# facebookresearch/audio2photoreal

Hardware: NVIDIA B200
Metric: motion-frames/sec full p_sample_loop (body, 1000 steps, T=600) (higher is better)
Workload: dtype bf16x2 split (fp32-equivalent), fp32 accumulate

## Files before the change

audio2photoreal_b200/csrc/engine.cu:

```cuda
#include <cuda_runtime.h>
#include <stdlib.h>
#include <map>
#include <string>
#include <vector>

#include "../../include/a2p_b200.h"
#include "attention_simt.cuh"
#include "common.cuh"
#include "elementwise.cuh"
#include "sgemm.cuh"
#include "umma_gemm.cuh"
#include "umma_attention.cuh"
#include "umma_chain.cuh"
#include "umma_attention2.cuh"
#include "umma_attention_short.cuh"

using namespace a2p;

namespace {

constexpr int MAXL = 16;
constexpr int TCN_PAD = 24;
const int TCN_DIL[6] = {1, 2, 3, 1, 2, 3};

struct AttnW { const float *in_w, *in_b, *out_w, *out_b; };
struct LayerW {
  AttnW sa, ca, c2;
  const float *l1w, *l1b, *l2w, *l2b;
  const float *n1w, *n1b, *n2w, *n2b, *n2aw, *n2ab, *n3w, *n3b;
};

struct CondSet {
  bool set = false;
  int Bc = 0, S = 0, S2 = 0;
  float* base = nullptr;
  const float* hidden = nullptr;
};

struct GraphKey {
  int B, T, kind, n_steps, clip, mask;
  const void *coeffs, *ts, *scale, *x, *pred, *noise, *ws;
  const void *kv0, *kv1;
  unsigned long long seed; long long row0; int rng;
  int units;
  int pipes;
  bool operator==(const GraphKey& o) const {
    return B == o.B && T == o.T && kind == o.kind && n_steps == o.n_steps && clip == o.clip && mask == o.mask &&
           coeffs == o.coeffs && ts == o.ts && scale == o.scale && x == o.x && pred == o.pred && noise == o.noise &&
           ws == o.ws && kv0 == o.kv0 && kv1 == o.kv1 && seed == o.seed && row0 == o.row0 && rng == o.rng && units == o.units && pipes == o.pipes;
  }
};

}

struct a2p_denoiser {
  a2p_model_cfg cfg{};
  int dh = 0, nf = 0;
  bool bound = false;
  LayerW lw[MAXL]{};
  const float *time_w1, *time_b1, *time_w2, *time_b2, *time_w3, *time_b3;
  const float *normc_w, *normc_b, *inp_w, *inp_b, *fin_w, *fin_b, *fconv_w, *fconv_b;
  struct EncLayerW { const float *n1w, *n1b, *n2w, *n2b, *in_w, *in_b, *out_w, *out_b, *l1w, *l1b, *l2w, *l2b; };
  struct EncW {
    const float *cp_w = nullptr, *cp_b = nullptr;
    const float *p0w = nullptr, *p0b = nullptr, *p1w = nullptr, *p1b = nullptr, *p3w = nullptr, *p3b = nullptr;
    const float *fp_w = nullptr, *fp_b = nullptr, *fn_w = nullptr, *fn_b = nullptr;
    EncLayerW enc[2]{};
    int feat_dim = 0;
    bool ok = false;
  } encw;
  const float* conv_b[6];
  const float* time_freqs;
  float *film_w = nullptr, *film_b = nullptr, *ttk_w = nullptr, *ttk_b = nullptr, *ttv_w = nullptr, *ttv_b = nullptr;
  float* conv_w[6]{};
  float* conv_t[6]{};
  float2* rope_tab = nullptr;
  std::map<const float*, __nv_bfloat16*> wplanes;
  std::map<const float*, long long> wnumel;
  int num_sms = 148;
  int attn_skew_ns = 0;
  CondSet cond[2];
  int64_t launches = 0;
  int64_t graph_nodes = 0;
  static constexpr int MAXG = 4;
  cudaGraphExec_t gexec[MAXG] = {};
  int n_gexec = 0;
  cudaStream_t group_stream[MAXG] = {};
  cudaEvent_t ev_gstart = nullptr, ev_gdone[MAXG] = {}, ev_gfork[MAXG] = {};
  cudaStream_t cap_stream = nullptr;
  static constexpr int MAXU = 8;
  cudaStream_t cond_stream[MAXU] = {};
  cudaEvent_t ev_fork[MAXU] = {}, ev_join[MAXU] = {};
  cudaStream_t unit_stream[MAXU] = {};
  cudaEvent_t ev_ujoin[MAXU] = {};
  cudaEvent_t ev_bfork = nullptr;
  GraphKey gkey{};
  bool gvalid = false;
};

namespace {

struct PackedLayout {
  size_t film_w, film_b, ttk_w, ttk_b, ttv_w, ttv_b, conv_w[6], conv_t[6], rope, planes, planes_bytes, total;
};
size_t split_weight_elems(const a2p_model_cfg& c) {
  const size_t D = c.D, FF = c.FF, C = c.C;
  size_t per_layer = 2 * (3 * D * D + D * D) + 2 * FF * D + (c.fmt == A2P_FMT_POSE ? 4 * D * D : 0);
  size_t conv = 0;
  if (c.fmt == A2P_FMT_POSE) {
    const size_t cm = C > 256 ? C : 256;
    conv = 3 * (cm * C * 2 + C * C * 4) + C * C;
  }
  return per_layer * c.L + 2 * D * C + conv;
}
PackedLayout packed_layout(const a2p_model_cfg& c) {
  PackedLayout p{};
  size_t off = 0;
  auto take = [&](size_t nfloats) { size_t o = off; off = align_up(off + nfloats * 4, 256); return o; };
  const int nf = c.fmt == A2P_FMT_POSE ? 4 : 3;
  p.film_w = take((size_t)c.L * nf * 2 * c.D * c.D);
  p.film_b = take((size_t)c.L * nf * 2 * c.D);
  p.ttk_w = take((size_t)c.L * c.D * c.D);
  p.ttk_b = take((size_t)c.L * c.D);
  p.ttv_w = take((size_t)c.L * c.D * c.D);
  p.ttv_b = take((size_t)c.L * c.D);
  if (c.fmt == A2P_FMT_POSE) {
    const int cm = c.C > 256 ? c.C : 256;
    const int chans[6][2] = {{cm, c.C}, {c.C, cm}, {c.C, c.C}, {c.C, c.C}, {c.C, c.C}, {c.C, c.C}};
    for (int i = 0; i < 6; ++i) p.conv_w[i] = take((size_t)chans[i][0] * chans[i][1] * 3);
    for (int i = 0; i < 6; ++i) p.conv_t[i] = take((size_t)chans[i][0] * chans[i][1] * 3);
  }
  p.rope = take((size_t)c.max_pos * (c.D / 2) * 2);
  p.planes = off;
  p.planes_bytes = c.split_terms > 0 ? align_up(split_weight_elems(c) * 2 * c.split_terms + 64 * 256, 256) : 0;
  off += p.planes_bytes;
  p.total = off;
  return p;
}

struct KvLayout {
  size_t per_layer, ka, va, k2, v2, hidden, total;
  size_t kaP, vtaP, k2P, vt2P;
  size_t Sp, S2p;
};
KvLayout kv_layout(const a2p_model_cfg& c, int Bc, int S, int S2) {
  KvLayout k{};
  size_t a = (size_t)Bc * S * c.D, b = (size_t)Bc * S2 * c.D;
  k.ka = 0; k.va = a; k.k2 = 2 * a; k.v2 = 2 * a + b;
  k.per_layer = 2 * a + 2 * b;
  k.Sp = align_up((size_t)S, 8); k.S2p = align_up((size_t)(S2 > 0 ? S2 : 1), 8);
  if (c.split_terms > 0) {
    const size_t P = c.split_terms;
    auto take = [&](size_t bf16s) { size_t o = k.per_layer; k.per_layer += align_up(bf16s / 2 + 1, 64); return o; };
    k.per_layer = align_up(k.per_layer, 64);
    k.kaP = take(P * Bc * S * c.D);
    k.vtaP = take(P * c.D * Bc * k.Sp);
    k.k2P = take(P * (b ? b : 1));
    k.vt2P = take(P * c.D * Bc * k.S2p);
  }
  k.hidden = k.per_layer * c.L;
  k.total = k.hidden + (size_t)Bc * c.D;
  return k;
}

struct WsLayout {
  size_t counter, e, th, mt, ttok, tt, ttr, ktt, vtt, film, xin, x, h, hr, qkv, att, u, out, tcnA, tcnB, tcnC, total;
  size_t hP, hrP, attP, uP, xinP;
  size_t tcnUP, tcnVP;
// ... 160 lines not shown
const float* find(const std::map<std::string, std::pair<const float*, int64_t>>& m, const std::string& k, int64_t numel,
                  std::string& err) {
  auto it = m.find(k);
  if (it == m.end()) { if (err.empty()) err = "missing weight '" + k + "'"; return nullptr; }
  if (numel >= 0 && it->second.second != numel) {
    if (err.empty()) err = "weight '" + k + "' has " + std::to_string(it->second.second) + " elements, expected " + std::to_string(numel);
    return nullptr;
  }
  return it->second.first;
}

int attn2_variant() {
  static int v = -1;
  if (v < 0) v = getenv("A2P_ATTN2") ? atoi(getenv("A2P_ATTN2")) : 2;
  return v;
}

int branch_groups(int B) {
  const char* e = getenv("A2P_BRANCH_GROUPS");
  const int v = e ? atoi(e) : ((B >= 4 && B <= 16) ? 2 : 1);
  return v >= 4 ? 4 : (v >= 2 ? 2 : 1);
}
bool branch_streams_disabled() { return getenv("A2P_NO_BRANCH_STREAMS") != nullptr; }
int branch_stagger() {
  static int v = -1;
  if (v < 0) { const char* e = getenv("A2P_BRANCH_STAGGER"); v = e ? atoi(e) : 0; if (v < 0) v = 0; }
  return v;
}

int chain_priority() {
  static int v = 1 << 30;
  if (v == (1 << 30)) { const char* e = getenv("A2P_CHAIN_PRIO"); v = e ? atoi(e) : 0; }
  return v;
}

bool chain_disabled() {
  static int v = -1;
  if (v < 0) v = getenv("A2P_NO_CHAIN") ? 1 : 0;
  return v == 1;
}

int check_cfg(const a2p_model_cfg* c) {
  if (!c) A2P_FAIL("null cfg");
  if (c->fmt != A2P_FMT_POSE && c->fmt != A2P_FMT_FACE) A2P_FAIL("cfg.fmt must be 0 (pose) or 1 (face)");
  if (c->D != 256 && c->D != 512) A2P_FAIL("cfg.D=%d unsupported (256 or 512)", c->D);
  if (c->H <= 0 || c->D % c->H) A2P_FAIL("cfg.H=%d does not divide D=%d", c->H, c->D);
  int dh = c->D / c->H;
  if (dh != 32 && dh != 64) A2P_FAIL("head dim %d unsupported (32 or 64)", dh);
  if (c->L <= 0 || c->L > MAXL) A2P_FAIL("cfg.L=%d out of range", c->L);
  if (c->C % 8 || c->FF % 8) A2P_FAIL("cfg.C/FF must be multiples of 8");
  if (c->fmt == A2P_FMT_POSE && c->S2 <= 0) A2P_FAIL("pose needs S2 > 0");
  if (c->fmt == A2P_FMT_FACE && c->S2 != 0) A2P_FAIL("face must have S2 == 0");
  if (c->split_terms < 0 || c->split_terms > 3) A2P_FAIL("split_terms=%d must be 0 (exact fp32) or 1..3 bf16 planes", c->split_terms);
  if (c->max_pos < 2) A2P_FAIL("cfg.max_pos too small");
  return 0;
}

int forward_core(Ctx& c, int B, int T, const float* xin, const long long* ts, const int* counter, int mask, char* wsb,
                 const float** x0_cond, const float** x0_uncond, long long* x0_sample_stride, int b0 = 0, int B_total = 0) {
  if (B_total <= 0) B_total = B;
  a2p_denoiser* h = c.h;
  const a2p_model_cfg& cf = h->cfg;
  const int D = cf.D, L = cf.L, C = cf.C, nf = h->nf, H = cf.H, dh = h->dh;
  const int nb = (mask == A2P_MASK_BOTH) ? 2 : 1;
  const int R = nb * B;
  const int br0 = (mask == A2P_MASK_UNCOND) ? 1 : 0;
// ... 379 lines not shown
      a.V = a.K;
      a.V.base[0] = c0.base + k0.per_layer * l + k0.v2;
      a.V.base[1] = c1.base ? c1.base + k1.per_layer * l + k1.v2 : nullptr;
      a.kv_ld = D; a.S_main = S2; a.S_extra = 0;
      a.O = att; a.o_ld = D; a.o_sample_stride = sT; a.T = T; a.H = H; a.R = R; a.scale_log2e = scale_log2e;
      c.cat = CAT_ATT_CROSS2;
      c.begin(); A2P_TRY(launch_attn_simt(a, dh, st)); c.end();
      c.cat = CAT_PROJ;
      h->launches++;
      A2P_TRY(film_gemm(c, att, D, R * T, lw.c2.out_w, lw.c2.out_b, D, D, x, D, film, film_ld, fo + 2 * 2 * D, D, T));
    }
    c.cat = CAT_FFN;
    { int _c = c.cat; c.cat = CAT_LN; c.begin(); A2P_TRY(launch_ln_rope(D, x, D, lw.n3w, lw.n3b, hh, nullptr, D, h->rope_tab, T, 0, R * T, st)); c.end(); c.cat = _c; }
    h->launches++;
    A2P_TRY(gemm(c, hh, D, R * T, lw.l1w, D, lw.l1b, cf.FF, D, u, cf.FF, EPI_GELU));
    A2P_TRY(film_gemm(c, u, cf.FF, R * T, lw.l2w, lw.l2b, D, cf.FF, x, D, film, film_ld, fo + (nf - 1) * 2 * D, D, T));
  }
  c.cat = CAT_IO_TCN;
  if (P > 0 && cf.fmt == A2P_FMT_POSE) {
    const int cm = C > 256 ? C : 256;
    const int Pl = T + TCN_PAD, Mp = R * Pl;
    __nv_bfloat16* U = reinterpret_cast<__nv_bfloat16*>(wsb + w.tcnUP);
    __nv_bfloat16* V = reinterpret_cast<__nv_bfloat16*>(wsb + w.tcnVP);
    float *X = F(w.tcnA), *Y = F(w.tcnC);
    c.cat = CAT_IO_TCN;
    if (!chain) {
      A2P_TRY(launch_split_planes(P, x, D, hP, pstrideD, MT, D, 1.f, st));
      A2P_CUDA(cudaMemset2DAsync(U, (size_t)Pl * C * 2, 0, (size_t)TCN_PAD * C * 2, (size_t)P * R, st));
      h->launches += 2;
      TcGemmParams g{};
      g.Cp = U; g.cp_plane_stride = (long long)Mp * C; g.ldcp = C; g.remap_rps = T; g.remap_pad = TCN_PAD;
      A2P_TRY(tc_gemm(c, hP, MT, D, h->fin_w, 0, C, h->fin_b, TC_PLANES, g));
    }
    struct St { __nv_bfloat16* in; int cin; __nv_bfloat16* outp; int cout; float* f32; const float* skip; };
    St stg[6] = {{U, C, V, cm, nullptr, nullptr}, {V, cm, U, C, X, nullptr}, {U, C, V, C, Y, X},
                 {V, C, U, C, X, Y},              {U, C, V, C, Y, X},        {V, C, U, C, nullptr, Y}};
    for (int i = 0; i < 6; ++i) {
      TcGemmParams g{};
      g.taps = 3; g.dil = TCN_DIL[i]; g.slope = 0.2f;
      g.Cp = stg[i].outp; g.cp_plane_stride = (long long)Mp * stg[i].cout; g.ldcp = stg[i].cout;
      g.C = stg[i].f32; g.ldc = stg[i].cout;
      g.skip = stg[i].skip; g.ldskip = stg[i].cout;
      A2P_TRY(tc_gemm(c, stg[i].in, Mp, stg[i].cin, h->conv_t[i], 0, stg[i].cout, h->conv_b[i], TC_LRELU_PLANES, g));
    }
    {
      TcGemmParams g{};
      g.C = Y; g.ldc = C;
      A2P_TRY(tc_gemm(c, U, Mp, C, h->fconv_w, 0, C, h->fconv_b, TC_F32, g));
    }
    *x0_sample_stride = (long long)Pl * C;
    const float* o0 = Y + (size_t)TCN_PAD * C;
    *x0_cond = (mask & A2P_MASK_COND) ? o0 : nullptr;
    *x0_uncond = (mask == A2P_MASK_BOTH) ? o0 + (size_t)B * Pl * C : (mask == A2P_MASK_UNCOND ? o0 : nullptr);
    return 0;
  }
  if (P > 0) {
    A2P_TRY(launch_split_planes(P, x, D, hP, pstrideD, MT, D, 1.f, st));
    h->launches++;
    TcGemmParams g{};
    g.C = out; g.ldc = C;
    A2P_TRY(tc_gemm(c, hP, MT, D, h->fin_w, 0, C, h->fin_b, TC_F32, g));
  } else {
    A2P_TRY(gemm(c, x, D, R * T, h->fin_w, D, h->fin_b, C, D, out, C));
  }
  if (cf.fmt == A2P_FMT_POSE) {
    const int cm = C > 256 ? C : 256;
    const int P = T + TCN_PAD;
    float *A = F(w.tcnA), *Bf = F(w.tcnB), *Cc = F(w.tcnC);
    long long total = (long long)R * P * (C / 4);
    pad_copy_kernel<<<(unsigned)((total + 255) / 256), 256, 0, st>>>(out, A, T, TCN_PAD, C / 4, total);
    h->launches++;
    struct Stage { const float* in; int cin; float* outp; int cout; bool skip; };
    Stage stg[6] = {{A, C, Bf, cm, false}, {Bf, cm, A, C, false}, {A, C, Cc, C, true},
                    {Cc, C, A, C, true},   {A, C, Cc, C, true},   {Cc, C, A, C, true}};
    for (int i = 0; i < 6; ++i) {
      GemmParams ex{};
      ex.taps = 3; ex.dil = TCN_DIL[i]; ex.Kc = stg[i].cin; ex.slope = 0.2f;
      ex.skip = stg[i].in; ex.ldskip = stg[i].cin;
      const bool skip = stg[i].skip && stg[i].cin == stg[i].cout;
      A2P_TRY(gemm(c, stg[i].in, stg[i].cin, R * P, h->conv_w[i], 3LL * stg[i].cin, h->conv_b[i], stg[i].cout, 3 * stg[i].cin,
                   stg[i].outp, stg[i].cout, skip ? EPI_LRELU_SKIPAVG : EPI_LRELU, &ex));
// ... 183 lines not shown
      int tot = (int)(chans[i][0] * chans[i][1] * 3);
      permute_conv_w_kernel<<<ceil_div(tot, 256), 256, 0, st>>>(cw, h->conv_w[i], (int)chans[i][0], (int)chans[i][1]);
      permute_conv_w_tapmajor_kernel<<<ceil_div(tot, 256), 256, 0, st>>>(cw, h->conv_t[i], (int)chans[i][0], (int)chans[i][1]);
    }
    h->fconv_w = W("final_conv.weight", C * C); h->fconv_b = W("final_conv.bias", C);
  }
  if (!err.empty()) A2P_FAIL("bind_weights: %s", err.c_str());
  h->wplanes.clear(); h->wnumel.clear();
  if (cf.split_terms > 0) {
    __nv_bfloat16* cur = reinterpret_cast<__nv_bfloat16*>(pb + pl.planes);
    const __nv_bfloat16* endp = reinterpret_cast<__nv_bfloat16*>(pb + pl.planes + pl.planes_bytes);
    auto split_w = [&](const float* wsrc, long long rows, long long cols) -> int {
      const long long numel = rows * cols;
      if (cur + numel * cf.split_terms > endp) A2P_FAIL("bind_weights: plane arena overflow");
      A2P_TRY(launch_split_planes(cf.split_terms, wsrc, cols, cur, numel, rows, (int)cols, 1.f, st));
      h->wplanes[wsrc] = cur; h->wnumel[wsrc] = numel;
      cur += align_up((size_t)numel * cf.split_terms, 64);
      return 0;
    };
    for (int l = 0; l < cf.L; ++l) {
      const LayerW& lw = h->lw[l];
      A2P_TRY(split_w(lw.sa.in_w, 3 * D, D)); A2P_TRY(split_w(lw.sa.out_w, D, D));
      A2P_TRY(split_w(lw.ca.in_w, 3 * D, D)); A2P_TRY(split_w(lw.ca.out_w, D, D));
      if (cf.fmt == A2P_FMT_POSE) { A2P_TRY(split_w(lw.c2.in_w, 3 * D, D)); A2P_TRY(split_w(lw.c2.out_w, D, D)); }
      A2P_TRY(split_w(lw.l1w, FF, D)); A2P_TRY(split_w(lw.l2w, D, FF));
    }
    A2P_TRY(split_w(h->inp_w, D, C)); A2P_TRY(split_w(h->fin_w, C, D));
    if (cf.fmt == A2P_FMT_POSE) {
      const int64_t cm = C > 256 ? C : 256;
      const int64_t chans[6][2] = {{cm, C}, {C, cm}, {C, C}, {C, C}, {C, C}, {C, C}};
      for (int i = 0; i < 6; ++i) A2P_TRY(split_w(h->conv_t[i], 3 * chans[i][0], chans[i][1]));
      A2P_TRY(split_w(h->fconv_w, C, C));
    }
    A2P_TRY(init_umma_gemm());
    A2P_TRY(init_umma_attn());
    A2P_TRY(init_umma_chain());
    A2P_TRY(init_umma_attn2());
    A2P_TRY(init_umma_attn_short());
  }
  {
    int dev = 0;
    cudaGetDevice(&dev);
    cudaDeviceGetAttribute(&h->num_sms, cudaDevAttrMultiProcessorCount, dev);
  }
  rope_table_kernel<<<ceil_div(cf.max_pos * (int)(D / 2), 256), 256, 0, st>>>(freqs, h->rope_tab, cf.max_pos, (int)(D / 2));
  A2P_CUDA(cudaGetLastError());
  h->bound = true;
  h->gvalid = false;
  return 0;
}

size_t a2p_kv_cache_bytes(const a2p_model_cfg* cfg, int Bc, int S) {
  if (check_cfg(cfg) || Bc <= 0 || S <= 0) return 0;
  return kv_layout(*cfg, Bc, S, cfg->S2).total * sizeof(float);
}

size_t a2p_conditioning_workspace_bytes(const a2p_model_cfg* cfg, int Bc, int S) {
  if (check_cfg(cfg) || Bc <= 0 || S <= 0) return 0;
  const size_t D = cfg->D;
  return (2 * align_up((size_t)Bc * S * D, 64) + align_up((size_t)Bc * (cfg->S2 > 0 ? cfg->S2 : 1) * D, 64)) * sizeof(float) + 512;
}

size_t a2p_workspace_bytes(const a2p_model_cfg* cfg, int B, int T) {
  if (check_cfg(cfg) || B <= 0 || T <= 0) return 0;
  const size_t one = ws_layout(*cfg, B, T).total;
  if (!(cfg->split_terms == 2 && cfg->D == 256)) return one;
// ... 486 lines not shown
```

audio2photoreal_b200/csrc/testing.cu:

```cuda
#include <cuda_runtime.h>
#include <stdlib.h>
#include <string>
#include <vector>

#include "../../include/a2p_b200.h"
#include "attention_simt.cuh"
#include "common.cuh"
#include "elementwise.cuh"
#include "sgemm.cuh"
#include "umma_gemm.cuh"
#include "umma_attention.cuh"
#include "umma_chain.cuh"
#include "umma_attention2.cuh"
#include "umma_attention_short.cuh"
#include "umma_microbench.cuh"
#include "../../include/a2p_b200_testing.h"

using namespace a2p;

extern "C" {

const char* a2p_test_last_error(void) { return a2p::last_error().c_str(); }

size_t a2p_test_tc_gemm_scratch_bytes(int M, int N, int K, int taps) {
  return ((size_t)3 * M * K + (size_t)3 * taps * N * K) * 2 + 1024;
}

int a2p_test_tc_gemm(int terms, int M, int N, int K, int taps, int dil, const float* A, const float* W, const float* bias,
                     float* C, void* scratch, size_t scratch_bytes, int iters, float* ms_out, void* stream) {
  if (scratch_bytes < a2p_test_tc_gemm_scratch_bytes(M, N, K, taps)) A2P_FAIL("test_tc_gemm: scratch too small");
  cudaStream_t st = (cudaStream_t)stream;
  A2P_TRY(init_umma_gemm());
  int dev = 0, sms = 148;
  cudaGetDevice(&dev);
  cudaDeviceGetAttribute(&sms, cudaDevAttrMultiProcessorCount, dev);
  __nv_bfloat16* Ap = (__nv_bfloat16*)scratch;
  __nv_bfloat16* Wp = Ap + align_up((size_t)3 * M * K, 64);
  A2P_TRY(launch_split_planes(terms, A, K, Ap, (long long)M * K, M, K, 1.f, st));
  A2P_TRY(launch_split_planes(terms, W, K, Wp, (long long)taps * N * K, (long long)taps * N, K, 1.f, st));
  TcOperands o{Ap, K, (long long)M * K, Wp, K, (long long)N * K};
  TcGemmParams p{};
  p.M = M; p.N = N; p.K = K; p.taps = taps; p.dil = dil; p.bias = bias; p.C = C; p.ldc = N; p.out_scale = 1.f;
  A2P_TRY(launch_umma_gemm(terms, o, p, TC_F32, sms, st));
  cudaEvent_t e0, e1;
  cudaEventCreate(&e0); cudaEventCreate(&e1);
  cudaEventRecord(e0, st);
  for (int i = 0; i < iters; ++i) A2P_TRY(launch_umma_gemm(terms, o, p, TC_F32, sms, st));
  cudaEventRecord(e1, st);
// ... 197 lines not shown
  cudaEvent_t e0, e1;
  cudaEventCreate(&e0); cudaEventCreate(&e1);
  cudaEventRecord(e0, st);
  for (int i = 0; i < iters; ++i) A2P_TRY(launch_attn_simt(a, dh, st));
  cudaEventRecord(e1, st);
  A2P_CUDA(cudaStreamSynchronize(st));
  float ms = 0.f;
  cudaEventElapsedTime(&ms, e0, e1);
  if (ms_out) *ms_out = iters > 0 ? ms / iters : 0.f;
  cudaEventDestroy(e0); cudaEventDestroy(e1);
  return 0;
}

int a2p_test_sgemm(int M, int N, int K, int taps, int dil, const float* A, const float* W, const float* bias, float* C,
                   int iters, float* ms_out, void* stream) {
  cudaStream_t st = (cudaStream_t)stream;
  GemmParams p{};
  p.A = A; p.lda = K; p.W = W; p.ldw = (long long)taps * K; p.bias = bias; p.C = C; p.ldc = N; p.M = M; p.N = N; p.K = taps * K;
  p.taps = taps; p.dil = dil; p.Kc = K; p.epi = EPI_BIAS;
  A2P_TRY(launch_sgemm(p, st));
  cudaEvent_t e0, e1;
  cudaEventCreate(&e0); cudaEventCreate(&e1);
  cudaEventRecord(e0, st);
  for (int i = 0; i < iters; ++i) A2P_TRY(launch_sgemm(p, st));
  cudaEventRecord(e1, st);
  A2P_CUDA(cudaStreamSynchronize(st));
  float ms = 0.f;
  cudaEventElapsedTime(&ms, e0, e1);
  if (ms_out) *ms_out = iters > 0 ? ms / iters : 0.f;
  cudaEventDestroy(e0); cudaEventDestroy(e1);
  return 0;
}

}
```

audio2photoreal_b200/csrc/umma.cuh:

```cuda
#pragma once
#include <cuda.h>
#include <cuda_bf16.h>
#include <cuda_runtime.h>
#include <stdint.h>

#include "common.cuh"

namespace a2p {
namespace umma {

__device__ __forceinline__ uint32_t smem_u32(const void* p) { return (uint32_t)__cvta_generic_to_shared(p); }

__device__ __forceinline__ void mbar_init(uint64_t* bar, uint32_t count) {
  asm volatile("mbarrier.init.shared::cta.b64 [%0], %1;" ::"r"(smem_u32(bar)), "r"(count));
}
__device__ __forceinline__ void fence_barrier_init() { asm volatile("fence.mbarrier_init.release.cluster;" ::: "memory"); }
__device__ __forceinline__ void fence_proxy_async() { asm volatile("fence.proxy.async.shared::cta;" ::: "memory"); }
__device__ __forceinline__ void mbar_expect_tx(uint64_t* bar, uint32_t bytes) {
  asm volatile("mbarrier.arrive.expect_tx.shared::cta.b64 _, [%0], %1;" ::"r"(smem_u32(bar)), "r"(bytes) : "memory");
}
__device__ __forceinline__ void mbar_arrive(uint64_t* bar) {
  asm volatile("mbarrier.arrive.shared::cta.b64 _, [%0];" ::"r"(smem_u32(bar)) : "memory");
}
__device__ __forceinline__ bool mbar_try_wait(uint64_t* bar, uint32_t parity) {
// ... 55 lines not shown
}
__device__ __forceinline__ void tma_load_3d_hint(const CUtensorMap* m, uint64_t* bar, void* dst, int c0, int c1, int c2, uint64_t pol) {
  asm volatile(
      "cp.async.bulk.tensor.3d.shared::cluster.global.mbarrier::complete_tx::bytes.L2::cache_hint [%0], [%1, {%3, %4, %5}], [%2], %6;"
      ::"r"(smem_u32(dst)), "l"(reinterpret_cast<uint64_t>(m)), "r"(smem_u32(bar)), "r"(c0), "r"(c1), "r"(c2), "l"(pol)
      : "memory");
}

template <int NCOLS>
__device__ __forceinline__ void tmem_alloc(uint32_t* slot_in_smem) {
  asm volatile("tcgen05.alloc.cta_group::1.sync.aligned.shared::cta.b32 [%0], %1;" ::"r"(smem_u32(slot_in_smem)), "n"(NCOLS));
  asm volatile("tcgen05.relinquish_alloc_permit.cta_group::1.sync.aligned;");
}
template <int NCOLS>
__device__ __forceinline__ void tmem_dealloc(uint32_t taddr) {
  asm volatile("tcgen05.dealloc.cta_group::1.sync.aligned.b32 %0, %1;" ::"r"(taddr), "n"(NCOLS));
}
__device__ __forceinline__ void fence_before() { asm volatile("tcgen05.fence::before_thread_sync;" ::: "memory"); }
__device__ __forceinline__ void fence_after() { asm volatile("tcgen05.fence::after_thread_sync;" ::: "memory"); }

__device__ __forceinline__ void tmem_ld32(uint32_t taddr, float* v) {
  uint32_t* r = reinterpret_cast<uint32_t*>(v);
  asm volatile(
      "tcgen05.ld.sync.aligned.32x32b.x32.b32 "
      "{%0, %1, %2, %3, %4, %5, %6, %7, %8, %9, %10, %11, %12, %13, %14, %15, "
      "%16, %17, %18, %19, %20, %21, %22, %23, %24, %25, %26, %27, %28, %29, %30, %31}, [%32];"
      : "=r"(r[0]), "=r"(r[1]), "=r"(r[2]), "=r"(r[3]), "=r"(r[4]), "=r"(r[5]), "=r"(r[6]), "=r"(r[7]), "=r"(r[8]),
        "=r"(r[9]), "=r"(r[10]), "=r"(r[11]), "=r"(r[12]), "=r"(r[13]), "=r"(r[14]), "=r"(r[15]), "=r"(r[16]),
        "=r"(r[17]), "=r"(r[18]), "=r"(r[19]), "=r"(r[20]), "=r"(r[21]), "=r"(r[22]), "=r"(r[23]), "=r"(r[24]),
        "=r"(r[25]), "=r"(r[26]), "=r"(r[27]), "=r"(r[28]), "=r"(r[29]), "=r"(r[30]), "=r"(r[31])
      : "r"(taddr));
}
__device__ __forceinline__ void tmem_ld_wait() { asm volatile("tcgen05.wait::ld.sync.aligned;" ::: "memory"); }

__device__ __forceinline__ uint64_t smem_desc_sw128(uint32_t saddr) {
  uint64_t d = 0;
  d |= (uint64_t)((saddr >> 4) & 0x3FFF);
  d |= (uint64_t)1 << 16;
  d |= (uint64_t)(1024 >> 4) << 32;
  d |= (uint64_t)1 << 46;
  d |= (uint64_t)2 << 61;
  return d;
}
constexpr uint32_t kDescHiSw128 = (uint32_t)(1024 >> 4) | (1u << 14) | (2u << 29);
__device__ __forceinline__ uint32_t desc_lo(uint32_t saddr) { return ((saddr >> 4) & 0x3FFFu) | (1u << 16); }
__device__ __forceinline__ uint64_t desc_make(uint32_t lo) { return ((uint64_t)kDescHiSw128 << 32) | (uint64_t)lo; }

__device__ __forceinline__ uint64_t smem_desc_sw64(uint32_t saddr) {
  uint64_t d = 0;
  d |= (uint64_t)((saddr >> 4) & 0x3FFF);
  d |= (uint64_t)1 << 16;
  d |= (uint64_t)(512 >> 4) << 32;
  d |= (uint64_t)1 << 46;
  d |= (uint64_t)4 << 61;
  return d;
}
__host__ __device__ constexpr uint32_t idesc_bf16_f32(int M, int N) {
  return (1u << 4) | (1u << 7) | (1u << 10) | ((uint32_t)(N >> 3) << 17) | ((uint32_t)(M >> 4) << 24);
}
__device__ __forceinline__ void mma_bf16(uint32_t tmem_d, uint64_t adesc, uint64_t bdesc, uint32_t idesc, uint32_t accumulate) {
  asm volatile(
      "{\n\t.reg .pred p;\n\t"
      "setp.ne.b32 p, %4, 0;\n\t"
      "tcgen05.mma.cta_group::1.kind::f16 [%0], %1, %2, %3, p;\n\t}"
      ::"r"(tmem_d), "l"(adesc), "l"(bdesc), "r"(idesc), "r"(accumulate)
      : "memory");
}
__device__ __forceinline__ void mma_commit(uint64_t* bar) {
  asm volatile("tcgen05.commit.cta_group::1.mbarrier::arrive::one.shared::cluster.b64 [%0];" ::"r"(smem_u32(bar)) : "memory");
}

__device__ __forceinline__ bool elect_one() {
  uint32_t pred;
  asm volatile(
      "{\n\t.reg .pred p;\n\t"
      "elect.sync _|p, 0xffffffff;\n\t"
      "selp.u32 %0, 1, 0, p;\n\t}"
      : "=r"(pred));
  return pred != 0;
}

template <int P>
__device__ __forceinline__ void split_bf16(float x, __nv_bfloat16* out) {
  float r = x;
#pragma unroll
  for (int i = 0; i < P; ++i) {
    __nv_bfloat16 b = __float2bfloat16_rn(r);
    out[i] = b;
    r = r - __bfloat162float(b);
// ... 50 lines not shown
```

include/a2p_b200_testing.h:

```cpp
#ifndef A2P_B200_TESTING_H
#define A2P_B200_TESTING_H
#include <stddef.h>
#include <stdint.h>
#ifdef __cplusplus
extern "C" {
#endif

const char* a2p_test_last_error(void);

size_t a2p_test_tc_gemm_scratch_bytes(int M, int N, int K, int taps);
int a2p_test_tc_gemm(int terms, int M, int N, int K, int taps, int dil, const float* A, const float* W, const float* bias,
                     float* C, void* scratch, size_t scratch_bytes, int iters, float* ms_out, void* stream);
int a2p_test_sgemm(int M, int N, int K, int taps, int dil, const float* A, const float* W, const float* bias, float* C,
                   int iters, float* ms_out, void* stream);

size_t a2p_test_tc_attention_scratch_bytes(int R, int T, int D, int S, int n_extra);
int a2p_test_tc_attention(int terms, int R, int T, int D, int dh, int S, int n_extra, const float* Q, const float* K,
                          const float* V, const float* Kx, const float* Vx, float* O, void* scratch, size_t scratch_bytes,
                          int iters, float* ms_out, void* stream);
void a2p_test_attn2_set_persist(int on);
int a2p_test_simt_attention(int R, int T, int D, int dh, int S, int n_extra, const float* Q, const float* K, const float* V,
                            const float* Kx, const float* Vx, float* O, int iters, float* ms_out, void* stream);

size_t a2p_test_chain_scratch_bytes(int M, int K0, int N1, int T);
void a2p_test_chain_set_mode(int cl);
void a2p_test_chain_set_nsplit(int n);
int a2p_test_chain_nsplit_policy(int tiles, int n_acc, int concurrent, int K0);
int a2p_test_chain(int M, int T, int K0, int N1, int film_mode, int ln_mode, int rope, int gelu, int vjob, float out_scale,
                   int scale_ncols, const float* A0, const float* W0, const float* bias0, const float* film, float* x,
                   const float* ln_w, const float* ln_b, const float* rope_freqs, const float* W1, const float* bias1,
                   const float* W2, const float* bias2, void* Cp_out, void* Vt_out, void* scratch, size_t scratch_bytes,
                   int iters, float* ms_out, void* stream);

void a2p_test_philox(uint32_t c0, uint32_t c1, uint32_t c2, uint32_t c3, uint32_t k0, uint32_t k1, uint32_t* out4);

int a2p_test_mma_rate(int N, int a_from_tmem, int n_mma, long long* cycles_out_dev, void* stream);

int a2p_test_tmem_ldst_rate(int store, int n_ops, int n_warps, long long* cycles_out_dev, void* stream);

#ifdef __cplusplus
}
#endif
#endif
```

Measured before the change: 2903.

## Fuse the six dilated TCN conv layers and final conv into one UMMA kernel

After: 2978 (median of 6 runs). 2.6% higher.

```diff
diff --git a/audio2photoreal_b200/csrc/engine.cu b/audio2photoreal_b200/csrc/engine.cu
--- a/audio2photoreal_b200/csrc/engine.cu
+++ b/audio2photoreal_b200/csrc/engine.cu
@@ -14,6 +14,7 @@
 #include "umma_chain.cuh"
 #include "umma_attention2.cuh"
 #include "umma_attention_short.cuh"
+#include "umma_tcn.cuh"
 
 using namespace a2p;
 
@@ -74,6 +75,7 @@
   float *film_w = nullptr, *film_b = nullptr, *ttk_w = nullptr, *ttk_b = nullptr, *ttv_w = nullptr, *ttv_b = nullptr;
   float* conv_w[6]{};
   float* conv_t[6]{};
+  const uint8_t* tcn_w = nullptr;
   float2* rope_tab = nullptr;
   std::map<const float*, __nv_bfloat16*> wplanes;
   std::map<const float*, long long> wnumel;
@@ -101,8 +103,10 @@
 namespace {
 
 struct PackedLayout {
-  size_t film_w, film_b, ttk_w, ttk_b, ttv_w, ttv_b, conv_w[6], conv_t[6], rope, planes, planes_bytes, total;
+  size_t film_w, film_b, ttk_w, ttk_b, ttv_w, ttv_b, conv_w[6], conv_t[6], rope, planes, planes_bytes, tcnw, total;
 };
+bool tcn_fused_supported(const a2p_model_cfg& c) { return c.fmt == A2P_FMT_POSE && c.split_terms == 2 && c.C <= TCN_CP; }
+
 size_t split_weight_elems(const a2p_model_cfg& c) {
   const size_t D = c.D, FF = c.FF, C = c.C;
   size_t per_layer = 2 * (3 * D * D + D * D) + 2 * FF * D + (c.fmt == A2P_FMT_POSE ? 4 * D * D : 0);
@@ -134,6 +138,8 @@
   p.planes = off;
   p.planes_bytes = c.split_terms > 0 ? align_up(split_weight_elems(c) * 2 * c.split_terms + 64 * 256, 256) : 0;
   off += p.planes_bytes;
+  p.tcnw = 0;
+  if (tcn_fused_supported(c)) { p.tcnw = off; off += align_up(tcn_w_bytes(), 256); }
   p.total = off;
   return p;
 }
@@ -360,6 +366,11 @@
   static int v = 1 << 30;
   if (v == (1 << 30)) { const char* e = getenv("A2P_CHAIN_PRIO"); v = e ? atoi(e) : 0; }
   return v;
+}
+
+bool tcn_fused_enabled() {
+  const char* e = getenv("A2P_TCN_FUSED");
+  return !e || atoi(e) != 0;
 }
 
 bool chain_disabled() {
@@ -805,6 +816,18 @@
       g.Cp = U; g.cp_plane_stride = (long long)Mp * C; g.ldcp = C; g.remap_rps = T; g.remap_pad = TCN_PAD;
       A2P_TRY(tc_gemm(c, hP, MT, D, h->fin_w, 0, C, h->fin_b, TC_PLANES, g));
     }
+    if (chain && h->tcn_w && tcn_fused_enabled()) {
+      TcnParams tp{};
+      tp.U = U; tp.u_plane_stride = (long long)Mp * C; tp.W = h->tcn_w;
+      for (int i = 0; i < 6; ++i) tp.bias[i] = h->conv_b[i];
+      tp.bias[6] = h->fconv_b;
+      tp.Y = Y; tp.T = T; tp.C = C;
+      h->launches++;
+      if (c.prof) c.tag = "umma_tcn";
+      c.begin();
+      A2P_TRY(launch_umma_tcn(tp, R, st));
+      c.end();
+    } else {
     struct St { __nv_bfloat16* in; int cin; __nv_bfloat16* outp; int cout; float* f32; const float* skip; };
     St stg[6] = {{U, C, V, cm, nullptr, nullptr}, {V, cm, U, C, X, nullptr}, {U, C, V, C, Y, X},
                  {V, C, U, C, X, Y},              {U, C, V, C, Y, X},        {V, C, U, C, nullptr, Y}};
@@ -820,6 +843,7 @@
       TcGemmParams g{};
       g.C = Y; g.ldc = C;
       A2P_TRY(tc_gemm(c, U, Mp, C, h->fconv_w, 0, C, h->fconv_b, TC_F32, g));
+    }
     }
     *x0_sample_stride = (long long)Pl * C;
     const float* o0 = Y + (size_t)TCN_PAD * C;
@@ -1069,6 +1093,16 @@
       for (int i = 0; i < 6; ++i) A2P_TRY(split_w(h->conv_t[i], 3 * chans[i][0], chans[i][1]));
       A2P_TRY(split_w(h->fconv_w, C, C));
     }
+    h->tcn_w = nullptr;
+    if (tcn_fused_supported(cf)) {
+      const __nv_bfloat16* src[7];
+      long long ps[7];
+      for (int i = 0; i < 6; ++i) { src[i] = h->wplanes[h->conv_t[i]]; ps[i] = h->wnumel[h->conv_t[i]]; }
+      src[6] = h->wplanes[h->fconv_w]; ps[6] = h->wnumel[h->fconv_w];
+      A2P_TRY(pack_tcn_weights(src, ps, C, reinterpret_cast<uint8_t*>(pb + pl.tcnw), st));
+      h->tcn_w = reinterpret_cast<const uint8_t*>(pb + pl.tcnw);
+      A2P_TRY(init_umma_tcn());
+    }
     A2P_TRY(init_umma_gemm());
     A2P_TRY(init_umma_attn());
     A2P_TRY(init_umma_chain());
diff --git a/audio2photoreal_b200/csrc/testing.cu b/audio2photoreal_b200/csrc/testing.cu
--- a/audio2photoreal_b200/csrc/testing.cu
+++ b/audio2photoreal_b200/csrc/testing.cu
@@ -14,6 +14,7 @@
 #include "umma_attention2.cuh"
 #include "umma_attention_short.cuh"
 #include "umma_microbench.cuh"
+#include "umma_tcn.cuh"
 #include "../../include/a2p_b200_testing.h"
 
 using namespace a2p;
@@ -277,4 +278,92 @@
   return 0;
 }
 
-}
+static int g_tcn_fused = 1;
+void a2p_test_tcn_set_fused(int on) { g_tcn_fused = on != 0; }
+
+int a2p_test_tcn(int R, int T, int C, const float* X, const float* const* w, const float* const* b, float* Y_out, int iters,
+                 float* ms_out, void* stream) {
+  cudaStream_t st = (cudaStream_t)stream;
+  if (C > TCN_CP || C % 8) A2P_FAIL("test_tcn: C=%d", C);
+  A2P_TRY(init_umma_gemm());
+  A2P_TRY(init_umma_tcn());
+  int dev = 0, sms = 148;
+  cudaGetDevice(&dev);
+  cudaDeviceGetAttribute(&sms, cudaDevAttrMultiProcessorCount, dev);
+  const int cm = 256, Pl = T + TCN_HALO;
+  const long long Mp = (long long)R * Pl;
+  const int cout[7] = {cm, C, C, C, C, C, C}, cin[7] = {C, cm, C, C, C, C, C}, taps[7] = {3, 3, 3, 3, 3, 3, 1};
+  std::vector<void*> bufs;
+  auto alloc = [&](size_t bytes) -> void* { void* q = nullptr; if (cudaMalloc(&q, bytes) != cudaSuccess) return nullptr; bufs.push_back(q); return q; };
+  auto run = [&]() -> int {
+    __nv_bfloat16* U = (__nv_bfloat16*)alloc((size_t)2 * Mp * cm * 2);
+    __nv_bfloat16* V = (__nv_bfloat16*)alloc((size_t)2 * Mp * cm * 2);
+    float* Xf = (float*)alloc((size_t)Mp * cm * 4);
+    float* Yf = (float*)alloc((size_t)Mp * cm * 4);
+    uint8_t* Wpk = (uint8_t*)alloc(tcn_w_bytes());
+    const __nv_bfloat16* Wp[7];
+    long long ps[7];
+    for (int l = 0; l < 7; ++l) {
+      ps[l] = (long long)taps[l] * cout[l] * cin[l];
+      __nv_bfloat16* q = (__nv_bfloat16*)alloc((size_t)2 * ps[l] * 2);
+      if (!q) A2P_FAIL("test_tcn: cudaMalloc failed");
+      A2P_TRY(launch_split_planes(2, w[l], cin[l], q, ps[l], (long long)taps[l] * cout[l], cin[l], 1.f, st));
+      Wp[l] = q;
+    }
+    if (!U || !V || !Xf || !Yf || !Wpk) A2P_FAIL("test_tcn: cudaMalloc failed");
+    A2P_CUDA(cudaMemsetAsync(U, 0, (size_t)2 * Mp * C * 2, st));
+    A2P_CUDA(cudaMemsetAsync(Yf, 0, (size_t)Mp * C * 4, st));
+    for (int r = 0; r < R; ++r)
+      A2P_TRY(launch_split_planes(2, X + (size_t)r * T * C, C, U + ((size_t)r * Pl + TCN_HALO) * C, Mp * C, T, C, 1.f, st));
+    A2P_TRY(pack_tcn_weights(Wp, ps, C, Wpk, st));
+    auto launch = [&]() -> int {
+      if (g_tcn_fused) {
+        TcnParams tp{};
+        tp.U = U; tp.u_plane_stride = Mp * C; tp.W = Wpk;
+        for (int l = 0; l < 7; ++l) tp.bias[l] = b[l];
+        tp.Y = Yf; tp.T = T; tp.C = C;
+        return launch_umma_tcn(tp, R, st);
+      }
+      struct St { __nv_bfloat16* in; __nv_bfloat16* outp; float* f32; const float* skip; };
+      St stg[6] = {{U, V, nullptr, nullptr}, {V, U, Xf, nullptr}, {U, V, Yf, Xf}, {V, U, Xf, Yf}, {U, V, Yf, Xf}, {V, U, nullptr, Yf}};
+      for (int i = 0; i < 7; ++i) {
+        TcGemmParams g{};
+        g.M = (int)Mp; g.N = cout[i]; g.K = cin[i]; g.taps = taps[i]; g.dil = tcn_dil(i); g.bias = b[i]; g.out_scale = 1.f;
+        TcOperands o{i < 6 ? stg[i].in : U, cin[i], Mp * cin[i], Wp[i], cin[i], (long long)cout[i] * cin[i]};
+        if (i < 6) {
+          g.slope = 0.2f; g.Cp = stg[i].outp; g.cp_plane_stride = Mp * cout[i]; g.ldcp = cout[i];
+          g.C = stg[i].f32; g.ldc = cout[i]; g.skip = stg[i].skip; g.ldskip = cout[i];
+          A2P_TRY(launch_umma_gemm(2, o, g, TC_LRELU_PLANES, sms, st));
+        } else {
+          g.C = Yf; g.ldc = C;
+          A2P_TRY(launch_umma_gemm(2, o, g, TC_F32, sms, st));
+        }
+      }
+      return 0;
+    };
+    A2P_TRY(launch());
+    A2P_CUDA(cudaMemcpy2DAsync(Y_out, (size_t)T * C * 4, Yf + (size_t)TCN_HALO * C, (size_t)Pl * C * 4, (size_t)T * C * 4, R,
+                               cudaMemcpyDeviceToDevice, st));
+    A2P_CUDA(cudaStreamSynchronize(st));
+    if (ms_out) *ms_out = 0.f;
+    if (iters <= 0) return 0;
+    for (int i = 0; i < 3; ++i) A2P_TRY(launch());
+    cudaEvent_t e0, e1;
+    cudaEventCreate(&e0); cudaEventCreate(&e1);
+    cudaEventRecord(e0, st);
+    for (int i = 0; i < iters; ++i) A2P_TRY(launch());
+    cudaEventRecord(e1, st);
+    A2P_CUDA(cudaStreamSynchronize(st));
+    float ms = 0.f;
+    cudaEventElapsedTime(&ms, e0, e1);
+    if (ms_out) *ms_out = ms / iters;
+    cudaEventDestroy(e0); cudaEventDestroy(e1);
+    return 0;
+  };
+  const int rc = run();
+  cudaStreamSynchronize(st);
+  for (void* q : bufs) cudaFree(q);
+  return rc;
+}
+
+}
diff --git a/audio2photoreal_b200/csrc/umma.cuh b/audio2photoreal_b200/csrc/umma.cuh
--- a/audio2photoreal_b200/csrc/umma.cuh
+++ b/audio2photoreal_b200/csrc/umma.cuh
@@ -111,6 +111,31 @@
       : "r"(taddr));
 }
 __device__ __forceinline__ void tmem_ld_wait() { asm volatile("tcgen05.wait::ld.sync.aligned;" ::: "memory"); }
+__device__ __forceinline__ void tmem_ld16(uint32_t taddr, float* v) {
+  uint32_t* r = reinterpret_cast<uint32_t*>(v);
+  asm volatile(
+      "tcgen05.ld.sync.aligned.32x32b.x16.b32 "
+      "{%0, %1, %2, %3, %4, %5, %6, %7, %8, %9, %10, %11, %12, %13, %14, %15}, [%16];"
+      : "=r"(r[0]), "=r"(r[1]), "=r"(r[2]), "=r"(r[3]), "=r"(r[4]), "=r"(r[5]), "=r"(r[6]), "=r"(r[7]), "=r"(r[8]),
+        "=r"(r[9]), "=r"(r[10]), "=r"(r[11]), "=r"(r[12]), "=r"(r[13]), "=r"(r[14]), "=r"(r[15])
+      : "r"(taddr));
+}
+__device__ __forceinline__ void tmem_st16(uint32_t taddr, const float* v) {
+  const uint32_t* r = reinterpret_cast<const uint32_t*>(v);
+  asm volatile(
+      "tcgen05.st.sync.aligned.32x32b.x16.b32 [%0], "
+      "{%1, %2, %3, %4, %5, %6, %7, %8, %9, %10, %11, %12, %13, %14, %15, %16};"
+      ::"r"(taddr), "r"(r[0]), "r"(r[1]), "r"(r[2]), "r"(r[3]), "r"(r[4]), "r"(r[5]), "r"(r[6]), "r"(r[7]), "r"(r[8]),
+        "r"(r[9]), "r"(r[10]), "r"(r[11]), "r"(r[12]), "r"(r[13]), "r"(r[14]), "r"(r[15])
+      : "memory");
+}
+__device__ __forceinline__ void tmem_st_wait() { asm volatile("tcgen05.wait::st.sync.aligned;" ::: "memory"); }
+
+__device__ __forceinline__ void bulk_load(void* dst, const void* src, uint32_t bytes, uint64_t* bar) {
+  asm volatile("cp.async.bulk.shared::cluster.global.mbarrier::complete_tx::bytes [%0], [%1], %2, [%3];"
+               ::"r"(smem_u32(dst)), "l"(reinterpret_cast<uint64_t>(src)), "r"(bytes), "r"(smem_u32(bar))
+               : "memory");
+}
 
 __device__ __forceinline__ uint64_t smem_desc_sw128(uint32_t saddr) {
   uint64_t d = 0;
@@ -134,6 +159,12 @@
   d |= (uint64_t)4 << 61;
   return d;
 }
+constexpr uint32_t kDescHiNoSwz128 = (uint32_t)(128 >> 4) | (1u << 14);
+__device__ __forceinline__ uint32_t desc_lo_noswz(uint32_t saddr, uint32_t lbo_bytes) {
+  return ((saddr >> 4) & 0x3FFFu) | ((lbo_bytes >> 4) << 16);
+}
+__device__ __forceinline__ uint64_t desc_make_noswz(uint32_t lo) { return ((uint64_t)kDescHiNoSwz128 << 32) | (uint64_t)lo; }
+
 __host__ __device__ constexpr uint32_t idesc_bf16_f32(int M, int N) {
   return (1u << 4) | (1u << 7) | (1u << 10) | ((uint32_t)(N >> 3) << 17) | ((uint32_t)(M >> 4) << 24);
 }
diff --git a/audio2photoreal_b200/csrc/umma_tcn.cuh b/audio2photoreal_b200/csrc/umma_tcn.cuh
--- /dev/null
+++ b/audio2photoreal_b200/csrc/umma_tcn.cuh
@@ -0,0 +1,262 @@
+#pragma once
+#include <cuda_bf16.h>
+
+#include "common.cuh"
+#include "umma.cuh"
+#include "umma_gemm.cuh"
+
+namespace a2p {
+
+constexpr int TCN_WIN = 104;
+constexpr int TCN_HALO = 24;
+constexpr int TCN_G = 6;
+constexpr int TCN_ROWS = 128 + TCN_G;
+constexpr int TCN_CS = TCN_ROWS * 16;
+constexpr int TCN_CP = 112;
+constexpr int TCN_PS_S = (TCN_CP / 8) * TCN_CS, TCN_PS_L = (256 / 8) * TCN_CS;
+constexpr int TCN_S_OFF = 0, TCN_L_OFF = 2 * TCN_PS_S, TCN_RING_OFF = TCN_L_OFF + 2 * TCN_PS_L;
+constexpr int TCN_NST = 4, TCN_SLOT = 8192;
+constexpr int TCN_BAR_OFF = TCN_RING_OFF + TCN_NST * TCN_SLOT;
+constexpr int TCN_SMEM = TCN_BAR_OFF + 128;
+constexpr int TCN_SKIP_COL = 128;
+static_assert(TCN_SMEM <= 232448, "umma_tcn: shared memory");
+
+__host__ __device__ constexpr int tcn_kch(int l) { return l == 1 ? 16 : 7; }
+__host__ __device__ constexpr int tcn_taps(int l) { return l == 6 ? 1 : 3; }
+__host__ __device__ constexpr int tcn_dil(int l) { return l == 6 ? 0 : l % 3 + 1; }
+__host__ __device__ constexpr int tcn_nhalf(int l) { return l == 0 ? 2 : 1; }
+__host__ __device__ constexpr int tcn_nu(int l) { return l == 0 ? 128 : TCN_CP; }
+__host__ __device__ constexpr int tcn_units(int l) { return tcn_kch(l) * tcn_taps(l) * tcn_nhalf(l); }
+__host__ __device__ constexpr int tcn_unit_bytes(int l) { return 64 * tcn_nu(l); }
+inline size_t tcn_w_bytes() {
+  size_t b = 0;
+  for (int l = 0; l < 7; ++l) b += (size_t)tcn_units(l) * tcn_unit_bytes(l);
+  return b;
+}
+
+struct TcnParams {
+  const __nv_bfloat16* U; long long u_plane_stride;
+  const uint8_t* W;
+  const float* bias[7];
+  float* Y;
+  int T, C, n_win;
+};
+
+template <int L>
+__device__ __forceinline__ void tcn_epilogue(const TcnParams& p, uint8_t* smem, uint32_t trow, int m, int cgrp, int s, int t0) {
+  constexpr int NCOL = L == 0 ? 256 : TCN_CP;
+  constexpr bool SKIP_IN = L >= 2 && L <= 5, SKIP_OUT = L >= 1 && L <= 4;
+  constexpr int PSO = (L & 1) ? TCN_PS_S : TCN_PS_L;
+  uint8_t* out = smem + ((L & 1) ? TCN_S_OFF : TCN_L_OFF) + 16 * (TCN_G + m);
+  const int cout = L == 0 ? 256 : p.C;
+  const float* bias = p.bias[L];
+  const int Pl = p.T + TCN_HALO;
+#pragma unroll 1
+  for (int cc = cgrp; cc < NCOL / 16; cc += 2) {
+    float v[16], sk[16];
+    umma::tmem_ld16(trow + cc * 16, v);
+    if (SKIP_IN) umma::tmem_ld16(trow + TCN_SKIP_COL + cc * 16, sk);
+    umma::tmem_ld_wait();
+#pragma unroll
+    for (int i = 0; i < 16; ++i) {
+      const int col = cc * 16 + i;
+      float o = v[i] + (col < cout ? __ldg(bias + col) : 0.f);
+      if (L < 6) {
+        o = o > 0.f ? o : o * 0.2f;
+        if (SKIP_IN) o = (sk[i] + o) / 2.0f;
+      }
+      v[i] = o;
+    }
+    if (SKIP_OUT) umma::tmem_st16(trow + TCN_SKIP_COL + cc * 16, v);
+    if (L < 6) {
+#pragma unroll
+      for (int g = 0; g < 2; ++g) {
+        uint32_t p0[4], p1[4];
+#pragma unroll
+        for (int e = 0; e < 4; ++e) {
+          uint32_t sp[2];
+          umma::split_bf16_pair<2>(v[8 * g + 2 * e], v[8 * g + 2 * e + 1], sp);
+          p0[e] = sp[0]; p1[e] = sp[1];
+        }
+        uint8_t* dst = out + (2 * cc + g) * TCN_CS;
+        *reinterpret_cast<uint4*>(dst) = make_uint4(p0[0], p0[1], p0[2], p0[3]);
+        *reinterpret_cast<uint4*>(dst + PSO) = make_uint4(p1[0], p1[1], p1[2], p1[3]);
+      }
+    } else {
+      const int pr = t0 + m;
+      if (m >= TCN_HALO && pr < Pl) {
+        float* y = p.Y + ((long long)s * Pl + pr) * p.C;
+#pragma unroll
+        for (int g = 0; g < 4; ++g) {
+          const int col = cc * 16 + 4 * g;
+          if (col < p.C) *reinterpret_cast<float4*>(y + col) = make_float4(v[4 * g], v[4 * g + 1], v[4 * g + 2], v[4 * g + 3]);
+        }
+      }
+    }
+  }
+  if (SKIP_OUT) umma::tmem_st_wait();
+}
+
+template <int L>
+__device__ __forceinline__ void tcn_epilogue_step(const TcnParams& p, uint8_t* smem, uint64_t* accf, uint64_t* actr, uint32_t trow,
+                                                  int m, int cgrp, int s, int t0) {
+  umma::mbar_wait(accf, L & 1);
+  umma::fence_after();
+  tcn_epilogue<L>(p, smem, trow, m, cgrp, s, t0);
+  if (L < 6) {
+    umma::fence_proxy_async();
+    umma::fence_before();
+    umma::mbar_arrive(actr);
+  }
+}
+
+__global__ void __launch_bounds__(384, 1) umma_tcn_kernel(const __grid_constant__ TcnParams p) {
+  extern __shared__ __align__(16) uint8_t tcn_smem[];
+  uint8_t* smem = tcn_smem;
+  uint64_t* bars = reinterpret_cast<uint64_t*>(smem + TCN_BAR_OFF);
+  uint64_t* full = bars;
+  uint64_t* empty = bars + TCN_NST;
+  uint64_t* accf = bars + 2 * TCN_NST;
+  uint64_t* actr = accf + 1;
+  uint32_t* tmem_slot = reinterpret_cast<uint32_t*>(actr + 1);
+
+  const int warp = threadIdx.x >> 5, lane = threadIdx.x & 31;
+  const int s = blockIdx.x / p.n_win, t0 = (blockIdx.x - s * p.n_win) * TCN_WIN;
+
+  if (warp == 1 && lane == 0) {
+    for (int i = 0; i < TCN_NST; ++i) { umma::mbar_init(&full[i], 1); umma::mbar_init(&empty[i], 1); }
+    umma::mbar_init(accf, 1);
+    umma::mbar_init(actr, 256);
+    umma::fence_barrier_init();
+  }
+  if (warp == 2) umma::tmem_alloc<256>(tmem_slot);
+  umma::fence_before();
+  __syncthreads();
+  umma::fence_after();
+  const uint32_t tmem_base = *tmem_slot;
+
+  if (warp == 0) {
+    int stage = 0; uint32_t phase = 0;
+    const uint8_t* src = p.W;
+    for (int l = 0; l < 7; ++l) {
+      const uint32_t ub = tcn_unit_bytes(l);
+      for (int u = 0; u < tcn_units(l); ++u) {
+        umma::mbar_wait(&empty[stage], phase ^ 1);
+        if (umma::elect_one()) {
+          umma::mbar_expect_tx(&full[stage], ub);
+          umma::bulk_load(smem + TCN_RING_OFF + stage * TCN_SLOT, src, ub, &full[stage]);
+        }
+        __syncwarp();
+        src += ub;
+        if (++stage == TCN_NST) { stage = 0; phase ^= 1; }
+      }
+    }
+    pdl_trigger();
+  } else if (warp == 1) {
+    const uint32_t sbase = umma::smem_u32(smem);
+    int stage = 0; uint32_t phase = 0;
+    for (int l = 0; l < 7; ++l) {
+      const int kch = tcn_kch(l), taps = tcn_taps(l), dil = tcn_dil(l), nh = tcn_nhalf(l), nu = tcn_nu(l);
+      const uint32_t idesc = umma::idesc_bf16_f32(128, nu);
+      const uint32_t abase = sbase + ((l & 1) ? TCN_L_OFF : TCN_S_OFF) + 16 * TCN_G;
+      const uint32_t aps = (l & 1) ? TCN_PS_L : TCN_PS_S;
+      umma::mbar_wait(actr, l & 1);
+      umma::fence_after();
+      for (int c = 0; c < kch; ++c)
+        for (int j = 0; j < taps; ++j)
+          for (int h = 0; h < nh; ++h) {
+            umma::mbar_wait(&full[stage], phase);
+            umma::fence_after();
+            if (umma::elect_one()) {
+              const uint32_t a0 = abase + 2 * c * TCN_CS - 16 * (taps - 1 - j) * dil;
+              const uint32_t b0 = sbase + TCN_RING_OFF + stage * TCN_SLOT;
+#pragma unroll
+              for (int pr = 0; pr < 3; ++pr)
+                umma::mma_bf16(tmem_base + h * 128,
+                               umma::desc_make_noswz(umma::desc_lo_noswz(a0 + prod_a(pr) * aps, TCN_CS)),
+                               umma::desc_make_noswz(umma::desc_lo_noswz(b0 + prod_b(pr) * 32 * nu, 16 * nu)), idesc,
+                               (c | j | pr) != 0 ? 1u : 0u);
+              umma::mma_commit(&empty[stage]);
+            }
+            __syncwarp();
+            if (++stage == TCN_NST) { stage = 0; phase ^= 1; }
+          }
+      if (umma::elect_one()) umma::mma_commit(accf);
+      __syncwarp();
+    }
+  } else if (warp >= 4) {
+    const int et = threadIdx.x - 128;
+    const int q = warp & 3, cgrp = (warp - 4) >> 2, m = q * 32 + lane;
+    const int Pl = p.T + TCN_HALO;
+    pdl_wait();
+    for (int idx = et; idx < 2 * (TCN_CP / 8) * TCN_ROWS; idx += 256) {
+      const int i = idx % TCN_ROWS, ch = (idx / TCN_ROWS) % (TCN_CP / 8), pl = idx / (TCN_ROWS * (TCN_CP / 8));
+      const int pr = t0 - TCN_G + i;
+      uint4 v = make_uint4(0u, 0u, 0u, 0u);
+      if (pr >= 0 && pr < Pl && ch * 8 < p.C)
+        v = __ldg(reinterpret_cast<const uint4*>(p.U + pl * p.u_plane_stride + ((long long)s * Pl + pr) * p.C + ch * 8));
+      *reinterpret_cast<uint4*>(smem + TCN_S_OFF + pl * TCN_PS_S + ch * TCN_CS + 16 * i) = v;
+    }
+    for (int idx = et; idx < 2 * 32 * TCN_G; idx += 256) {
+      const int i = idx % TCN_G, ch = (idx / TCN_G) % 32, pl = idx / (TCN_G * 32);
+      *reinterpret_cast<uint4*>(smem + TCN_L_OFF + pl * TCN_PS_L + ch * TCN_CS + 16 * i) = make_uint4(0u, 0u, 0u, 0u);
+    }
+    umma::fence_proxy_async();
+    umma::mbar_arrive(actr);
+    const uint32_t trow = tmem_base + ((uint32_t)(q * 32) << 16);
+    tcn_epilogue_step<0>(p, smem, accf, actr, trow, m, cgrp, s, t0);
+    tcn_epilogue_step<1>(p, smem, accf, actr, trow, m, cgrp, s, t0);
+    tcn_epilogue_step<2>(p, smem, accf, actr, trow, m, cgrp, s, t0);
+    tcn_epilogue_step<3>(p, smem, accf, actr, trow, m, cgrp, s, t0);
+    tcn_epilogue_step<4>(p, smem, accf, actr, trow, m, cgrp, s, t0);
+    tcn_epilogue_step<5>(p, smem, accf, actr, trow, m, cgrp, s, t0);
+    tcn_epilogue_step<6>(p, smem, accf, actr, trow, m, cgrp, s, t0);
+  }
+  umma::fence_before();
+  __syncthreads();
+  if (warp == 2) {
+    umma::fence_after();
+    umma::tmem_dealloc<256>(tmem_base);
+  }
+}
+
+__global__ void pack_tcn_layer_kernel(const __nv_bfloat16* __restrict__ src, long long ps, int taps, int nh, int nu, int Cout,
+                                      int Cin, __nv_bfloat16* __restrict__ dst, long long total) {
+  const long long idx = (long long)blockIdx.x * blockDim.x + threadIdx.x;
+  if (idx >= total) return;
+  const int e = (int)(idx % 8), n = (int)((idx / 8) % nu), kk = (int)((idx / (8 * nu)) % 2), q = (int)((idx / (16 * nu)) % 2);
+  const int u = (int)(idx / (32 * nu));
+  const int c = u / (taps * nh), j = (u / nh) % taps, h = u % nh;
+  const int co = h * 128 + n, k = c * 16 + kk * 8 + e;
+  dst[idx] = (co < Cout && k < Cin) ? src[q * ps + ((long long)j * Cout + co) * Cin + k] : __float2bfloat16(0.f);
+}
+
+inline int pack_tcn_weights(const __nv_bfloat16* const conv[7], const long long plane_stride[7], int C, uint8_t* dst, cudaStream_t st) {
+  if (C > TCN_CP) A2P_FAIL("umma_tcn: C=%d > %d", C, TCN_CP);
+  for (int l = 0; l < 7; ++l) {
+    const int cout = l == 0 ? 256 : C, cin = l == 1 ? 256 : C;
+    const long long total = (long long)tcn_units(l) * tcn_unit_bytes(l) / 2;
+    pack_tcn_layer_kernel<<<(unsigned)((total + 255) / 256), 256, 0, st>>>(conv[l], plane_stride[l], tcn_taps(l), tcn_nhalf(l),
+                                                                            tcn_nu(l), cout, cin, reinterpret_cast<__nv_bfloat16*>(dst), total);
+    A2P_CUDA(cudaGetLastError());
+    dst += total * 2;
+  }
+  return 0;
+}
+
+inline int init_umma_tcn() {
+  A2P_CUDA(cudaFuncSetAttribute(umma_tcn_kernel, cudaFuncAttributeMaxDynamicSharedMemorySize, TCN_SMEM));
+  return 0;
+}
+
+inline int launch_umma_tcn(TcnParams p, int R, cudaStream_t st) {
+  if (p.C > TCN_CP || p.C % 8) A2P_FAIL("umma_tcn: C=%d must be a multiple of 8 and <= %d", p.C, TCN_CP);
+  if ((reinterpret_cast<uintptr_t>(p.U) | (reinterpret_cast<uintptr_t>(p.W)) | (reinterpret_cast<uintptr_t>(p.Y))) % 16 ||
+      (p.u_plane_stride * 2) % 16)
+    A2P_FAIL("umma_tcn: operands not 16-byte aligned");
+  p.n_win = ceil_div(p.T, TCN_WIN);
+  A2P_CUDA(launch_pdl(umma_tcn_kernel, dim3(R * p.n_win), dim3(384), (size_t)TCN_SMEM, st, p));
+  return 0;
+}
+
+}
diff --git a/include/a2p_b200_testing.h b/include/a2p_b200_testing.h
--- a/include/a2p_b200_testing.h
+++ b/include/a2p_b200_testing.h
@@ -32,6 +32,10 @@
                    const float* W2, const float* bias2, void* Cp_out, void* Vt_out, void* scratch, size_t scratch_bytes,
                    int iters, float* ms_out, void* stream);
 
+void a2p_test_tcn_set_fused(int on);
+int a2p_test_tcn(int R, int T, int C, const float* X, const float* const* w, const float* const* b, float* Y_out, int iters,
+                 float* ms_out, void* stream);
+
 void a2p_test_philox(uint32_t c0, uint32_t c1, uint32_t c2, uint32_t c3, uint32_t k0, uint32_t k1, uint32_t* out4);
 
 int a2p_test_mma_rate(int N, int a_from_tmem, int n_mma, long long* cycles_out_dev, void* stream);
```
